# zhuhaozh/metadrive_ped

Measured on AMD Instinct MI355X. Metric: agent-steps/sec at 4096 envs x 240-beam lidar, higher is better.
Workload: dtype f32; 1 GPU; BASELINE configs[1]: 4096 batched MetaDriveEnv per GPU, 3-block PG map (reference default block distribution: curves, straights, ramps, X/T intersections, roundabouts), 240-beam lidar, traffic_density=0.1, trigger traffic, auto-reset; envs_per_gpu=4096, agents_per_env=1, mover_capacity=24, n_beams=240

## Files before the change

### metadrive_ped_amd/csrc/mdstep.hip

```cpp
#include <hip/hip_runtime.h>
#include <stddef.h>
#include <stdint.h>
#include <stdio.h>
#include <stdlib.h>

#include <type_traits>

#include "md_curriculum.h"
#include "md_expert.h"
#include "md_expert_sense.h"
#include "md_ai_protect.h"
#include "md_scenario.h"
#include "md_topdown.h"
#include "md_render.h"
#include "md_branch.h"
#include "md_ped.h"
#include "md_vector_obs.h"
#include "md_lean_pins.h"

namespace {

constexpr int kBlock = 256;

enum Phase : int {
    PH_RESET = 1,
    PH_IDM = 2,
    PH_INTEGRATE = 4,
    PH_LOCALIZE = 8,
    PH_CONTACTS = 16,
    PH_TRAFFIC = 32,
    PH_OBSERVE = 64,
    PH_LIDAR = 128,
    PH_LIFECYCLE = 256,
    PH_ALL = 511,
    PH_LOCALIZE_ROAD_FIRST = PH_LOCALIZE | (1 << 20),
};

thread_local char g_err[256] = "ok";

#ifdef MD_STAMP
__device__ unsigned long long* g_stamp_buf = nullptr;
__device__ const int* g_env_order = nullptr;
#define MD_STAMP_AT(i)                                                                         \
    do {                                                                                       \
        if (threadIdx.x == 0 && g_stamp_buf) {                                                 \
            unsigned long long* sb_ = g_stamp_buf + (size_t)blockIdx.x * 32;                   \
            sb_[(i)] = __builtin_readcyclecounter();                                           \
            if ((i) == 0) {                                                                    \
                sb_[12] = __builtin_amdgcn_s_memrealtime();                                    \
                sb_[14] = (unsigned long long)__builtin_amdgcn_s_getreg(63492) |               \
                          ((unsigned long long)__builtin_amdgcn_s_getreg(63508) << 32);        \
            }                                                                                  \
            if ((i) == 11) sb_[13] = __builtin_amdgcn_s_memrealtime();                         \
        }                                                                                      \
    } while (0)
#define MD_FINE_STAMP(cond, i)                                                                 \
    do {                                                                                       \
        if ((cond) && g_stamp_buf) g_stamp_buf[(size_t)blockIdx.x * 32 + 16 + (i)] = __builtin_readcyclecounter(); \
    } while (0)
#define MD_LOC_COUNT(cond, hit)                                                                \
    do {                                                                                       \
        if ((cond) && g_stamp_buf) {                                                           \
            atomicAdd(&g_stamp_buf[(size_t)blockIdx.x * 32 + 16 + 12], 1ull);                  \
            if (hit) atomicAdd(&g_stamp_buf[(size_t)blockIdx.x * 32 + 16 + 13], 1ull);         \
        }                                                                                      \
    } while (0)
#define MD_AHEAD_STAMP(cond, i)                                                                \
    do {                                                                                       \
        if ((cond) && g_stamp_buf) g_stamp_buf[(size_t)blockIdx.x * 32 + (i)] = __builtin_readcyclecounter(); \
    } while (0)
enum : int { MD_AHEAD_EVALUATED = 32, MD_AHEAD_HIT = 40, MD_AHEAD_MISS = 48 };
#define MD_AHEAD_COUNT(cond, what)                                                             \
    do {                                                                                       \
        if ((cond) && g_stamp_buf) atomicAdd(&g_stamp_buf[(size_t)blockIdx.x * 32 + 16 + 12], 1ull << (what)); \
    } while (0)
__device__ unsigned long long* g_contacts_buf = nullptr;
#define MD_CONTACTS_STAMP(cond, i)                                                             \
    do {                                                                                       \
        if ((cond) && g_contacts_buf) g_contacts_buf[(size_t)blockIdx.x * 8 + (i)] = __builtin_readcyclecounter(); \
    } while (0)
#define MD_CONTACTS_COUNT(cond, cells, items)                                                  \
    do {                                                                                       \
        if ((cond) && g_contacts_buf) {                                                        \
            g_contacts_buf[(size_t)blockIdx.x * 8 + 4] += (unsigned long long)(cells);         \
            g_contacts_buf[(size_t)blockIdx.x * 8 + 5] += (unsigned long long)(items);         \
        }                                                                                      \
    } while (0)
#else
#define MD_CONTACTS_STAMP(cond, i) do { } while (0)
#define MD_CONTACTS_COUNT(cond, cells, items) do { } while (0)
#define MD_STAMP_AT(i) do { } while (0)
#define MD_FINE_STAMP(cond, i) do { } while (0)
#define MD_LOC_COUNT(cond, hit) do { } while (0)
#define MD_AHEAD_STAMP(cond, i) do { } while (0)
#define MD_AHEAD_COUNT(cond, what) do { } while (0)
#endif
#ifndef MD_ENV_SKIP
#define MD_ENV_SKIP 0
#endif

__host__ __device__ constexpr uint32_t align_up(uint32_t b, uint32_t a) { return (b + a - 1) & ~(a - 1); }

__device__ __forceinline__ float bcast_f(float v, int src) { return __shfl(v, src, 64); }
__device__ __forceinline__ int bcast_i(int v, int src) { return __shfl(v, src, 64); }

__device__ __forceinline__ void wave_lds_sync() {
    __builtin_amdgcn_fence(__ATOMIC_RELEASE, "wavefront");
    __builtin_amdgcn_wave_barrier();
    __builtin_amdgcn_fence(__ATOMIC_ACQUIRE, "wavefront");
}

#ifndef MD_NT_STAGE
#define MD_NT_STAGE 1
#endif
typedef unsigned int md_u32x4 __attribute__((ext_vector_type(4)));
__device__ __forceinline__ uint4 ld_stream(const uint4* p) {
#if MD_NT_STAGE
    const md_u32x4 v = __builtin_nontemporal_load(reinterpret_cast<const md_u32x4*>(p));
    return make_uint4(v.x, v.y, v.z, v.w);
#else
    return *p;
#endif
}
__device__ __forceinline__ void st_stream(uint4* p, const uint4 v) {
#if MD_NT_STAGE
    md_u32x4 t;
    t.x = v.x; t.y = v.y; t.z = v.z; t.w = v.w;
    __builtin_nontemporal_store(t, reinterpret_cast<md_u32x4*>(p));
#else
    *p = v;
#endif
}
__device__ __forceinline__ void st_stream_f(float* p, float v) {
#if MD_NT_STAGE
    __builtin_nontemporal_store(v, p);
#else
    *p = v;
#endif
}

__device__ __forceinline__ int wave_min_i(int v, bool valid, int none) {
    unsigned long long m = __ballot(valid);
    int best = none;
    while (m) {
        const int l = __ffsll((long long)m) - 1;
        m &= m - 1;
        const int o = __shfl(v, l, 64);
        best = o < best ? o : best;
    }
    return best;
}

template <bool kLdsRow = false>
__device__ __forceinline__ void lidar_item(const MdWorld& w, const MdState& s, const MdConfig& c, int a, int sec, int lane,
                           float* __restrict__ out_row, unsigned long long* det) {
    const MdShape me = s.shape[a];
    const int beam = sec * 64 + lane;
    const bool valid = beam < c.n_beams;
    if (!md_present(me.flags)) {
        if (valid) out_row[beam] = 1.0f;
        return;
    }
    float bc = 1.0f, bs = 0.0f;
    if (valid) {
        bc = w.beam_cs[2 * beam];
        bs = w.beam_cs[2 * beam + 1];
    }
    const float dirx = (bc * me.c - bs * me.s) * c.lidar_range;
    const float diry = (bs * me.c + bc * me.s) * c.lidar_range;

    const int nb = min(64, c.n_beams - sec * 64);
// ... 272 lines not shown
        for (int fan = 0; fan < (f.n1 > 0 ? 2 : 1); ++fan) {
            const float* beam_cs = fan ? f.cs1 : f.cs0;
            const int n_beams = fan ? f.n1 : f.n0;
            const float reach = (fan ? f.range1 : f.range0) * 1.001f;
            const uint32_t kind_mask = fan ? f.mask1 : f.mask0;
            const float phase0 = fan ? ph1 : ph0;
            const bool uniform_fan = fan ? uni1 : uni0;
            const int beam_base = fan ? f.n0 : 0;
            const float inv_dphi = 1.0f / (6.283185307179586f / (float)n_beams);
            const float far = reach + rr;
            const bool near = in_reach && ((kind_mask >> b.kind) & 1u) && !(px * px + py * py > far * far);
            if (__ballot(near) == 0ull) continue;
            int i_lo = 0, n_try = n_beams;
            if (uniform_fan && near && n_beams > kAllBeamsMax)
                detector_beam_window(me, px, py, rr, phase0, inv_dphi, n_beams, i_lo, n_try);
            const int nt = near ? n_try : 0;
            int pin = nt;
#pragma unroll
            for (int off = 1; off < 64; off <<= 1) {
                const int v = __shfl_up(pin, off, 64);
                if (lane_id >= off) pin += v;
            }
            const int total = __shfl(pin, 63, 64);
            const int pex = pin - nt;
            for (int t0 = 0; t0 < total; t0 += 64) {
                const int t = t0 + lane_id;
                int l = 0;
#pragma unroll
                for (int step = 32; step >= 1; step >>= 1) {
                    const int cnd = l + step;
                    const int pc = __shfl(pex, cnd & 63, 64);
                    if (cnd < 64 && pc <= t) l = cnd;
                }
                const bool mine_ = t < total;
                const int k = t - __shfl(pex, l, 64);
                const float px_ = __shfl(px, l, 64), py_ = __shfl(py, l, 64), rr_ = __shfl(rr, l, 64);
                int i = __shfl(i_lo, l, 64) + k;
                if (i >= n_beams) i -= n_beams;
                if (!mine_) i = 0;
                const int q_ = __shfl(q0, l, 64);
                const float bc = beam_cs[2 * i], bs = beam_cs[2 * i + 1];
                const float ux = bc * me.c - bs * me.s, uy = bs * me.c + bc * me.s;
                const float perp = ux * py_ - uy * px_, along = ux * px_ + uy * py_;
                const bool pass = mine_ && !(md_fabs(perp) > rr_ * 1.001f + 1.0e-3f || along < -rr_ || along > reach + rr_);
                const unsigned long long m = __ballot(pass);
                if (m == 0ull) continue;
                if (cnt + 64 > kPairs) {
                    wave_lds_sync();
                    detector_drain2(w, me, f, pair_list, cnt, qa, lane_id);
                    __builtin_amdgcn_wave_barrier();
                    cnt = 0;
                }
                if (pass) pair_list[cnt + __popcll(m & ((1ull << lane_id) - 1ull))] = ((q_ - qa) << 8) | (beam_base + i);
                cnt += __popcll(m);
            }
        }
    }
    __builtin_amdgcn_wave_barrier();
    n_near = 0;
    };
    for (int q0 = qa; q0 < qb; q0 += 64) {
        const int q = q0 + lane_id;
        const QuadBall b = nb;
        if (q + 64 < qb) nb = quad_ball_of(w, q + 64);
        bool in_reach = false;
        if (q < qb) {
            const float px = b.mx - me.cx, py = b.my - me.cy;
            const float far = reach_max + b.rr;
            in_reach = !(px * px + py * py > far * far);
        }
        const unsigned long long m = __ballot(in_reach);
        if (m == 0ull) continue;
        if (n_near + 64 > kNear) work_off();
        if (in_reach) near_list[n_near + __popcll(m & ((1ull << lane_id) - 1ull))] = q - qa;
        n_near += __popcll(m);
        if (!across_rounds) work_off();
    }
    work_off();
    wave_lds_sync();
    detector_drain2(w, me, f, pair_list, cnt, qa, lane_id);
    __builtin_amdgcn_wave_barrier();
}

__device__ __host__ inline int detector_parts(int A) { return (A >= kBlock / 64) ? 1 : kBlock / 64; }
__device__ __host__ inline int detector_groups(int A) { return (A * detector_parts(A) + kBlock / 64 - 1) / (kBlock / 64); }

struct LineDetectorLds { uint32_t best, beams, pairs, bytes; };
__host__ __device__ inline LineDetectorLds line_detector_lds(int nb) {
    constexpr int kW = kBlock / 64;
    LineDetectorLds L;
    L.best = 0;
    L.beams = L.best + (uint32_t)kW * nb * sizeof(int);
    L.pairs = L.beams + (uint32_t)nb * 2 * sizeof(float);
    L.bytes = L.pairs + (uint32_t)kW * kDetPairs * sizeof(int);
    return L;
}

__global__ __launch_bounds__(kBlock) void line_detector_kernel(MdWorld w, MdState s, MdConfig c,
                                                               const float* __restrict__ beam_cs, int n_beams,
                                                               float range, uint32_t kind_mask, float* out,
                                                               int out_stride, int out_offset,
                                                               const float* __restrict__ beam_cs1, int n_beams1, float range1,
                                                               uint32_t kind_mask1, int out_offset1) {
    extern __shared__ __attribute__((aligned(16))) unsigned char smem[];
    constexpr int kW = kBlock / 64;
    const int A = c.agents_per_env;
    const int nb = n_beams + n_beams1;
    const int parts = detector_parts(A), groups = detector_groups(A);
    const LineDetectorLds L = line_detector_lds(nb);
    int* l_best = reinterpret_cast<int*>(smem + L.best);
    float* l_bm = reinterpret_cast<float*>(smem + L.beams);
    int* l_pairs = reinterpret_cast<int*>(smem + L.pairs);
    const int e = blockIdx.x / groups, grp = blockIdx.x - e * groups;
    if (e >= c.n_envs) return;
    const int tid = threadIdx.x, wave = tid >> 6, lane = tid & 63;
    const int m = w.env_map[e];
    const int q0 = w.quad_off[m], q1 = w.quad_off[m + 1];
    const int a_first = (grp * kW) / parts;
    const int n_here = min(A - a_first, kW / parts);
    for (int it = tid; it < n_here * nb; it += kBlock) l_best[it] = __float_as_int(1.0f);
    for (int it = tid; it < 2 * n_beams; it += kBlock) l_bm[it] = beam_cs[it];
    for (int it = tid; it < 2 * n_beams1; it += kBlock) l_bm[2 * n_beams + it] = beam_cs1[it];
    __syncthreads();
    const int per = (q1 - q0 + parts - 1) / parts;
    const int it = grp * kW + wave;
    if (it < A * parts) {
        const int a = it / parts, part = it - a * parts;
        const MdShape me = s.shape[e * c.cap + a];
        if (md_present(me.flags)) {
            const int qa = q0 + part * per, qb = min(qa + per, q1);
            DetFan2 f;
            f.cs0 = l_bm; f.n0 = n_beams; f.range0 = range; f.mask0 = kind_mask; f.best0 = l_best + (a - a_first) * nb;
            f.cs1 = l_bm + 2 * n_beams; f.n1 = n_beams1; f.range1 = range1; f.mask1 = kind_mask1; f.best1 = f.best0 + n_beams;
            detector_wave2(w, me, qa, qb, f, l_pairs + wave * kDetPairs, lane);
        }
    }
    __syncthreads();
    for (int k = tid; k < n_here * nb; k += kBlock) {
        const int al = k / nb, i = k - al * nb;
        float* row = out + (size_t)(e * A + a_first + al) * out_stride;
        if (i < n_beams) row[out_offset + i] = __int_as_float(l_best[k]);
        else row[out_offset1 + (i - n_beams)] = __int_as_float(l_best[k]);
    }
}

}

#include "parts/localize.inc"
#include "parts/contacts.inc"
#include "parts/idm.inc"
#include "parts/observe.inc"
#include "parts/trigger.inc"
#include "parts/lifecycle.inc"

namespace {

__device__ __forceinline__ void copy16(void* dst, const void* src, int nbytes, int tid, int nthreads) {
    uint4* d = reinterpret_cast<uint4*>(dst);
    const uint4* s = reinterpret_cast<const uint4*>(src);
    for (int i = tid; i < (nbytes >> 4); i += nthreads) d[i] = s[i];
}

constexpr int kStageMaxLanes = 64;
constexpr int kWideMaxEnvs = 640;
constexpr uint32_t kRemovedMark = 0xFFFFFFFFu;

__device__ __forceinline__ int kth_bit(unsigned long long lo, unsigned long long hi, int k) {
    int slot = -1;
    while (k >= 0) {
        if (lo) {
            slot = __ffsll((long long)lo) - 1;
            lo &= lo - 1;
        } else if (hi) {
            slot = 64 + __ffsll((long long)hi) - 1;
            hi &= hi - 1;
        } else {
            return -1;
        }
        --k;
    }
    return slot;
}

struct EnvImage {
    MdShape* shape;
    MdDyn* dyn;
    MdPid* pid;
    MdParam* param;
    MdNav* nav;
    float* action;
    uint32_t* flags;
    int32_t* final_lane;
};

__device__ __forceinline__ MdState local_view(const MdState& gv, const EnvImage& img) {
    MdState s = gv;
    s.shape = img.shape;
    s.dyn = img.dyn;
    s.nav = img.nav;
    s.pid = img.pid;
    s.action = img.action;
    s.flags = img.flags;
    s.param = img.param;
    s.final_lane = img.final_lane;
    return s;
}

struct SlotMask { unsigned long long lo, hi; };
static_assert(MD_MAX_CAP <= 128, "drive_mask: two 64-bit words per env");
__device__ __forceinline__ SlotMask drive_mask(const MdShape* shape, int cap, int lane) {
    SlotMask m = {0ull, 0ull};
    for (int j0 = 0; j0 < cap; j0 += 64) {
        const int j = j0 + lane;
        const unsigned long long mk = __ballot(j < cap && md_drives(shape[j < cap ? j : 0].flags));
        if (j0 == 0) m.lo = mk;
        else m.hi = mk;
    }
    return m;
}
__device__ __forceinline__ SlotMask agent_share(SlotMask m, int agents) {
    m.lo &= agents >= 64 ? ~0ull : ((1ull << agents) - 1ull);
    m.hi &= agents <= 64 ? 0ull : (agents >= 128 ? ~0ull : ((1ull << (agents - 64)) - 1ull));
    return m;
}
__device__ __forceinline__ int popc(SlotMask m) { return __popcll(m.lo) + __popcll(m.hi); }

#ifndef MD_ENV_BLOCK
#define MD_ENV_BLOCK 256
#endif
#ifndef MD_ENV_WAVES_EU
#define MD_ENV_WAVES_EU 7
#endif
__device__ __forceinline__ void lean_pins_fold(MdState& s, MdConfig& c) {
#define MD_PIN_ZERO(f) c.f = 0;
#define MD_PIN_NUL(p) s.p = nullptr;
    MD_LEAN_PINS(MD_PIN_ZERO, MD_PIN_NUL)
#undef MD_PIN_ZERO
#undef MD_PIN_NUL
}
__device__ __forceinline__ void lean_size_pins_fold(MdConfig& c, MdConfig& c_scan) {
#define MD_PIN_EQUALS(f, v) c.f = (v);
#define MD_PIN_AT_MOST(f, v)
    MD_LEAN_SIZE_PINS(MD_PIN_EQUALS, MD_PIN_AT_MOST)
#undef MD_PIN_EQUALS
#undef MD_PIN_AT_MOST
    c_scan = c;
#define MD_PIN_EQUALS(f, v)
#define MD_PIN_AT_MOST(f, v) c_scan.f = min(c.f, (v));
    MD_LEAN_SIZE_PINS(MD_PIN_EQUALS, MD_PIN_AT_MOST)
#undef MD_PIN_EQUALS
#undef MD_PIN_AT_MOST
}

template <int PH, bool RESPAWN, bool MULTI>
constexpr int env_waves_per_eu() { return (PH == PH_ALL && !RESPAWN && !MULTI && MD_ENV_BLOCK >= 128) ? MD_ENV_WAVES_EU : 0; }

struct EnvLds { uint32_t shape, dyn, nav, pid, action, flags, lanes, roads, scratch, param, final_lane, det, onlane, cfl, tk, bytes; };
__host__ __device__ inline EnvLds env_lds(int cap, int agents, int n_lanes, int n_roads, int waves, bool multi, bool lidar_only) {
    EnvLds L;
    L.shape = 0;
    L.dyn = L.shape + (uint32_t)cap * sizeof(MdShape);
    L.nav = L.dyn + (uint32_t)cap * sizeof(MdDyn);
    L.pid = L.nav + (uint32_t)cap * sizeof(MdNav);
    L.action = L.pid + (uint32_t)cap * sizeof(MdPid);
    L.flags = L.action + (uint32_t)cap * 2 * sizeof(float);
    L.lanes = align_up(L.flags + (uint32_t)cap * sizeof(uint32_t), 16);
    L.roads = L.lanes + (uint32_t)n_lanes * sizeof(MdLane);
    L.scratch = L.roads + (uint32_t)n_roads * sizeof(MdRoad);
    L.param = L.scratch + (uint32_t)waves * (multi ? kObsScratch : 48) * sizeof(float);
    L.final_lane = L.param + (uint32_t)cap * sizeof(MdParam);
    L.det = L.final_lane + align_up(cap, 2) * sizeof(int32_t);
    L.onlane = L.det + (uint32_t)agents * 2 * sizeof(unsigned long long);
    L.cfl = L.onlane + (uint32_t)cap * sizeof(uint32_t);
    const uint32_t shared_words = 2 * cap > 8 ? 2 * cap : 8;
    L.tk = L.onlane + shared_words * sizeof(uint32_t);
    L.bytes = lidar_only ? L.dyn : L.tk + 3 * sizeof(int);
    return L;
}

template <int PH, bool STAGE_MAP, bool RESPAWN = false, bool MULTI = false, int BLK = MD_ENV_BLOCK, bool NARROW = false>
__global__ __launch_bounds__(BLK)
__attribute__((amdgpu_waves_per_eu(env_waves_per_eu<PH, RESPAWN, MULTI>() ? env_waves_per_eu<PH, RESPAWN, MULTI>() : 1,
                                   env_waves_per_eu<PH, RESPAWN, MULTI>() ? env_waves_per_eu<PH, RESPAWN, MULTI>() : 8)))
void env_kernel(MdWorld w, MdState g, MdConfig c, float* lidar_out,
                                                  int lidar_stride, int lidar_offset) {
    constexpr int kBlock = BLK;
    constexpr int kWaves = kBlock / 64;
    constexpr bool kIdmKeys = !STAGE_MAP && !RESPAWN && !MULTI;
    constexpr bool kLocRoadFirst = PH == PH_ALL ? kIdmKeys : PH == PH_LOCALIZE_ROAD_FIRST;
    constexpr bool kObsLockstep = MD_OBS_LOCKSTEP && PH == PH_ALL && kIdmKeys;
    constexpr bool kObsAhead = MD_OBS_AHEAD && kObsLockstep && kWaves > 1;
    constexpr bool kContactsFlat = MD_CONTACTS_FLAT && PH == PH_ALL && kIdmKeys;
    if constexpr (PH == PH_ALL && !RESPAWN && !MULTI && !STAGE_MAP) lean_pins_fold(g, c);
    static_assert(!NARROW || (PH == PH_ALL && !RESPAWN && !MULTI && !STAGE_MAP), "NARROW: a form of the lean non-staged kernel only");
    MdConfig c_scan = c;
    if constexpr (NARROW) lean_size_pins_fold(c, c_scan);
    if ((int)blockIdx.x >= c.n_envs) return;
#ifdef MD_STAMP
    const int e = g_env_order ? g_env_order[blockIdx.x] : (int)blockIdx.x;
#else
    const int e = blockIdx.x;
#endif
    const int tid = threadIdx.x;
    const int wave = tid >> 6, lane = tid & 63;
    const int cap = c.cap;

    const int n_stage_lanes = STAGE_MAP ? w.max_lanes : 0, n_stage_roads = STAGE_MAP ? w.max_roads : 0;
    constexpr bool kLidarOnly = (PH == PH_LIDAR);
    const EnvLds L = env_lds(cap, c.agents_per_env, n_stage_lanes, n_stage_roads, kWaves, MULTI, kLidarOnly);
    extern __shared__ __attribute__((aligned(16))) unsigned char smem[];
    MdShape* l_shape = reinterpret_cast<MdShape*>(smem + L.shape);
    MdDyn* l_dyn = reinterpret_cast<MdDyn*>(smem + L.dyn);
    MdNav* l_nav = reinterpret_cast<MdNav*>(smem + L.nav);
    MdPid* l_pid = reinterpret_cast<MdPid*>(smem + L.pid);
    float* l_action = reinterpret_cast<float*>(smem + L.action);
    uint32_t* l_flags = reinterpret_cast<uint32_t*>(smem + L.flags);
    MdLane* l_lanes = reinterpret_cast<MdLane*>(smem + L.lanes);
    MdRoad* l_roads = reinterpret_cast<MdRoad*>(smem + L.roads);
    float* l_scratch = reinterpret_cast<float*>(smem + L.scratch) + wave * (MULTI ? kObsScratch : 48);
    MdParam* l_param = reinterpret_cast<MdParam*>(smem + L.param);
    int32_t* l_final = reinterpret_cast<int32_t*>(smem + L.final_lane);
    unsigned long long* l_det = reinterpret_cast<unsigned long long*>(smem + L.det);
    const EnvImage img = {l_shape, l_dyn, l_pid, l_param, l_nav, l_action, l_flags, l_final};
    uint32_t* l_onlane = reinterpret_cast<uint32_t*>(smem + L.onlane);
    uint32_t* l_cfl = reinterpret_cast<uint32_t*>(smem + L.cfl);
    int* l_tk = reinterpret_cast<int*>(smem + L.tk);
    const bool track_det = (PH == PH_ALL) && (RESPAWN || MULTI) && g.detected != nullptr;

    const MdState gv = md_env_view(&g, &c, e);
    const int reset_flag = (PH & PH_RESET) ? gv.need_reset[0] : 0;

    MD_STAMP_AT(0);
    const bool kFusedAct = (PH == PH_ALL) && gv.agent_action != nullptr;
    const MdLane* lanes;
    const MdRoad* roads;
    if (STAGE_MAP) {
        lanes = l_lanes;
        roads = l_roads;
    } else {
        lanes = w.lanes + w.lane_off[w.env_map[e]];
        roads = w.roads + w.road_off[w.env_map[e]];
    }
    if (kLidarOnly) {
        copy16(l_shape, gv.shape, cap * (int)sizeof(MdShape), tid, kBlock);
    } else if (kBlock >= 256) {
        const int n32 = cap * 2, n64 = cap * 4;
        const uint4* g_shape = reinterpret_cast<const uint4*>(gv.shape);
        const uint4* g_dyn = reinterpret_cast<const uint4*>(gv.dyn);
        const uint4* g_pid = reinterpret_cast<const uint4*>(gv.pid);
        const uint4* g_param = reinterpret_cast<const uint4*>(gv.param);
        const uint4* g_nav = reinterpret_cast<const uint4*>(gv.nav);
        uint4 r_shape, r_dyn, r_pid, r_param, r_nav0;
        float2 r_act;
        uint32_t r_fl;
        int r_fin;
        const bool p32 = tid < n32, pc = tid < cap;
        if (p32) {
            r_shape = ld_stream(&g_shape[tid]);
            r_dyn = ld_stream(&g_dyn[tid]);
            r_pid = ld_stream(&g_pid[tid]);
            r_param = ld_stream(&g_param[tid]);
        }
        if (tid < n64) r_nav0 = ld_stream(&g_nav[tid]);
        if (pc) {
            r_act = (kFusedAct && tid < c.agents_per_env) ? reinterpret_cast<const float2*>(gv.agent_action)[tid]
                                                          : reinterpret_cast<const float2*>(gv.action)[tid];
            r_fl = gv.flags[tid];
            r_fin = gv.final_lane ? gv.final_lane[tid] : 0;
        }
        if (STAGE_MAP) {
            const int m = w.env_map[e];
            const int lo = w.lane_off[m], ro = w.road_off[m];
            copy16(l_lanes, w.lanes + lo, (w.lane_off[m + 1] - lo) * (int)sizeof(MdLane), tid, kBlock);
            copy16(l_roads, w.roads + ro, (w.road_off[m + 1] - ro) * (int)sizeof(MdRoad), tid, kBlock);
        }
        if (p32) {
            reinterpret_cast<uint4*>(l_shape)[tid] = r_shape;
            reinterpret_cast<uint4*>(l_dyn)[tid] = r_dyn;
            reinterpret_cast<uint4*>(l_pid)[tid] = r_pid;
            reinterpret_cast<uint4*>(l_param)[tid] = r_param;
        }
        if (tid < n64) reinterpret_cast<uint4*>(l_nav)[tid] = r_nav0;
        for (int i = tid + kBlock; i < n64; i += kBlock) reinterpret_cast<uint4*>(l_nav)[i] = g_nav[i];
        if (pc) {
            reinterpret_cast<float2*>(l_action)[tid] = r_act;
            l_flags[tid] = r_fl;
            l_final[tid] = r_fin;
        }
        if (track_det)
            for (int j = tid; j < 2 * c.agents_per_env; j += kBlock) l_det[j] = 0ull;
    } else {
        copy16(l_shape, gv.shape, cap * (int)sizeof(MdShape), tid, kBlock);
        if (STAGE_MAP) {
            const int m = w.env_map[e];
            const int lo = w.lane_off[m], ro = w.road_off[m];
            copy16(l_lanes, w.lanes + lo, (w.lane_off[m + 1] - lo) * (int)sizeof(MdLane), tid, kBlock);
            copy16(l_roads, w.roads + ro, (w.road_off[m + 1] - ro) * (int)sizeof(MdRoad), tid, kBlock);
        }
        copy16(l_dyn, gv.dyn, cap * (int)sizeof(MdDyn), tid, kBlock);
        copy16(l_nav, gv.nav, cap * (int)sizeof(MdNav), tid, kBlock);
        copy16(l_pid, gv.pid, cap * (int)sizeof(MdPid), tid, kBlock);
        copy16(l_param, gv.param, cap * (int)sizeof(MdParam), tid, kBlock);
        for (int j = tid; j < cap; j += kBlock) {
            const float* src = (kFusedAct && j < c.agents_per_env) ? gv.agent_action : gv.action;
            l_action[2 * j] = src[2 * j];
            l_action[2 * j + 1] = src[2 * j + 1];
            l_flags[j] = gv.flags[j];
            l_final[j] = gv.final_lane ? gv.final_lane[j] : 0;
        }
        if (track_det)
            for (int j = tid; j < 2 * c.agents_per_env; j += kBlock) l_det[j] = 0ull;
    }
    const bool do_reset = reset_flag != 0;
    const int just_reset = do_reset ? 1 : 0;
    if (do_reset && !kLidarOnly) {
        __syncthreads();
        copy16(l_shape, gv.shape0, cap * (int)sizeof(MdShape), tid, kBlock);
        copy16(l_dyn, gv.dyn0, cap * (int)sizeof(MdDyn), tid, kBlock);
        copy16(l_nav, gv.nav0, cap * (int)sizeof(MdNav), tid, kBlock);
        copy16(l_pid, gv.pid0, cap * (int)sizeof(MdPid), tid, kBlock);
        if (MULTI && c.random_agent_model && gv.param0)
            copy16(l_param, gv.param0, cap * (int)sizeof(MdParam), tid, kBlock);
        for (int j = tid; j < cap; j += kBlock) {
            l_action[2 * j] = 0.0f;
            l_action[2 * j + 1] = 0.0f;
            l_flags[j] = 0u;
        }
        if (MULTI || (RESPAWN && (c.traffic_mode == 1 || c.traffic_mode == 2))) {
            for (int i = tid; i < cap * MD_ROUTE_LEN; i += kBlock) {
                gv.route_nodes[i] = gv.route_nodes0[i];
                gv.route_roads[i] = gv.route_roads0[i];
            }
            for (int j = tid; j < cap; j += kBlock) l_final[j] = gv.final_lane0[j];
        }
        if (MULTI) {
            for (int j = tid; j < cap; j += kBlock) gv.agent_id[j] = j;
            if (tid == 0) {
                gv.env_steps[0] = 0;
                int n0 = 0;
                for (int j = 0; j < c.agents_per_env; ++j) n0 += (gv.shape0[j].flags & MD_F_ALIVE) ? 1 : 0;
                gv.next_agent_id[0] = n0;
            }
        }
    }
    MdState s = local_view(gv, img);
    if (kLidarOnly) {
        s = gv;
        s.shape = l_shape;
    }
    if ((MULTI || PH == PH_ALL) && tid == 0) l_tk[0] = l_tk[1] = l_tk[2] = 0;
    if (kObsAhead && tid == 0) reinterpret_cast<int*>(smem + L.scratch)[kAhMark] = 0;
    __syncthreads();
    MD_STAMP_AT(1);
    constexpr bool kTriggerEarly = MD_TRIGGER_EARLY && PH == PH_ALL && kIdmKeys && kWaves > 1;
    constexpr int kTrigWord = (kWaves - 1) * 48 + 46;
    if (kTriggerEarly && wave == kWaves - 1) {
        int min_order, trig_road;
        trigger_search_wave(s, c_scan, lane, &min_order, &trig_road);
        if (lane == 0) {
            int* l_trig = reinterpret_cast<int*>(smem + L.scratch) + kTrigWord;
            l_trig[0] = min_order;
            l_trig[1] = trig_road;
        }
    }

    if ((PH & PH_LIFECYCLE) && MULTI && !just_reset) {
        lifecycle_block(w, s, c, w.env_map[e], tid, kBlock, reinterpret_cast<int*>(l_onlane));
    }

    constexpr bool kFused = (PH == PH_ALL);
    const bool agent_idm = (kFused && !RESPAWN && !MULTI) ? false : (c.agent_idm == MD_AGENT_IDM);
    const bool lane_change = (RESPAWN || MULTI) && c.agent_idm == MD_AGENT_LANE_CHANGE;
    constexpr bool kPlanAhead = kFused && kWaves > 1 && !MULTI;
    const bool plan_ahead = kPlanAhead && !agent_idm;
    if ((PH & PH_IDM) && !just_reset && !plan_ahead) {
        if (wave == 0) trigger_env(lanes, s, c, lane);
        __syncthreads();
        MD_STAMP_AT(2);
        for (int j = (agent_idm ? 0 : c.agents_per_env) + wave; j < cap; j += kWaves) {
            const int f = s.shape[j].flags;
            if (md_drives(f) && (agent_idm || !(f & MD_F_AGENT))) idm_vehicle_wave<kIdmKeys>(w, lanes, roads, s, c, w.env_map[e], j, lane, reinterpret_cast<int*>(l_scratch));
        }
        __syncthreads();
    }
    MD_STAMP_AT(3);
    if ((PH & PH_INTEGRATE) && !just_reset) {
        for (int j = tid; j < cap; j += kBlock) {
            if (lane_change && j < c.agents_per_env) {
                const int f = s.shape[j].flags;
                if (md_drives(f) && !(f & MD_F_SPAWNED)) md_lane_change_act(lanes, roads, &s, j);
            }
            if (RESPAWN) md_advance_mover(&s, &c, j);
            else md_integrate_mover(&s, &c, j);
        }
        if (!RESPAWN)
            for (int j = tid; j < cap; j += kBlock) md_walk_mover(&s, &c, j);
        __syncthreads();
    }
    MD_STAMP_AT(4);
    unsigned long long drv_lo = 0ull, drv_hi = 0ull;
    if (kFused) {
        const SlotMask drv = drive_mask(s.shape, cap, lane);
        drv_lo = drv.lo;
        drv_hi = NARROW ? 0ull : drv.hi;
        const SlotMask adrv = agent_share(drv, c.agents_per_env);
        const unsigned long long adrv_lo = adrv.lo, adrv_hi = NARROW ? 0ull : adrv.hi;
        const int nd = NARROW ? __popcll(drv_lo) : popc(drv), na = NARROW ? __popcll(adrv_lo) : popc(adrv);
        if (MULTI) {
            const int npair = (nd + 1) >> 1;
            for (int guard = 0; guard < npair + na; ++guard) {
                int item = 0;
                if (lane == 0) item = atomicAdd(&l_tk[0], 1);
                item = __builtin_amdgcn_readfirstlane(item);
                if (item < 0 || item >= npair + na) break;
                if (item < na) contacts_vehicle(w, s, c, e, kth_bit(adrv_lo, adrv_hi, item), lane, l_cfl);
                else localize_pair(w, lanes, roads, s, e, kth_bit(drv_lo, drv_hi, 2 * (item - na)), kth_bit(drv_lo, drv_hi, 2 * (item - na) + 1), lane, l_onlane);
            }
        } else if (nd + na <= kWaves) {
            for (int item = wave; item < nd + na; item += kWaves) {
                if (item < nd) {
                    if (!(MD_ENV_SKIP & 4)) localize_vehicle<kLocRoadFirst>(w, lanes, roads, s, e, kth_bit(drv_lo, drv_hi, item), lane, l_onlane);
                } else if (!(MD_ENV_SKIP & 8)) contacts_vehicle<kContactsFlat>(w, s, c, e, kth_bit(adrv_lo, adrv_hi, item - nd), lane, l_cfl);
            }
            if constexpr (kObsAhead) {
                if (nd + na < kWaves && wave == nd + na && !(MD_ENV_SKIP & 16))
                    observe_ahead_wave(lanes, roads, s, c, lane, reinterpret_cast<float*>(smem + L.scratch));
            }
        } else {
            const int npair = (nd + 1) >> 1;
            for (int item = wave; item < npair + na; item += kWaves) {
                if (item < npair) {
                    if (!(MD_ENV_SKIP & 4)) localize_pair<kLocRoadFirst>(w, lanes, roads, s, e, kth_bit(drv_lo, drv_hi, 2 * item), kth_bit(drv_lo, drv_hi, 2 * item + 1), lane, l_onlane);
                } else if (!(MD_ENV_SKIP & 8))
                    contacts_vehicle<kContactsFlat>(w, s, c, e, kth_bit(adrv_lo, adrv_hi, item - npair), lane, l_cfl);
            }
        }
        __syncthreads();
    } else {
        if (PH & PH_LOCALIZE) {
            for (int j = wave; j < cap; j += kWaves) localize_vehicle<kLocRoadFirst>(w, lanes, roads, s, e, j, lane);
            __syncthreads();
        }
        MD_STAMP_AT(5);
        if (PH & PH_CONTACTS) {
            for (int j = wave; j < cap; j += kWaves) contacts_vehicle(w, s, c, e, j, lane);
            __syncthreads();
        }
    }
    MD_STAMP_AT(6);
    if (PH & PH_TRAFFIC) {
        for (int j = tid; j < cap; j += kBlock) {
            const bool drove = kFused ? ((((j < 64) ? (drv_lo >> j) : (drv_hi >> (j - 64))) & 1ull) != 0ull) : false;
            if (kFused && !drove) continue;
            const int f = s.shape[j].flags;
            if (kFused)
                s.flags[j] = l_onlane[j] | ((f & MD_F_AGENT) ? l_cfl[j] : 0u);
            if (md_drives(f) && !(f & MD_F_AGENT) && !(s.flags[j] & MD_FL_ON_LANE)) {
                s.shape[j].flags = f & ~MD_F_ALIVE;
                if (kFused) l_cfl[j] = kRemovedMark;
            }
        }
        if (plan_ahead && wave == kWaves - 1) {
            if (kTriggerEarly) {
                const int* l_trig = reinterpret_cast<const int*>(smem + L.scratch) + kTrigWord;
                trigger_fire_wave(lanes, s, c_scan, lane, __builtin_amdgcn_readfirstlane(l_trig[0]), __builtin_amdgcn_readfirstlane(l_trig[1]));
            } else trigger_env(lanes, s, c_scan, lane);
        }
        __syncthreads();
        if (RESPAWN) {
            if (tid == 0) md_traffic_respawn_env(&w, lanes, &s, &c, w.env_map[e]);
            __syncthreads();
        }
    }
    MD_STAMP_AT(7);
    if (plan_ahead) {
        if (wave == 0) {
            if (!(MD_ENV_SKIP & 16))
                for (int a = 0; a < c.agents_per_env; ++a) observe_agent_wave1<kObsLockstep, kObsAhead>(lanes, roads, s, c, a, just_reset, lane, l_scratch);
        } else if (!(MD_ENV_SKIP & 2)) {
            int rank = 0;
            for (int j0 = 0; j0 < cap; j0 += 64) {
                const int jl = j0 + lane;
                const int fl = (jl < cap) ? s.shape[jl].flags : 0;
                unsigned long long mk = __ballot(jl < cap && md_drives(fl) && !(fl & MD_F_AGENT));
                while (mk) {
                    const int j = j0 + __ffsll((long long)mk) - 1;
                    mk &= mk - 1;
                    if (rank % (kWaves - 1) == wave - 1) idm_vehicle_wave<kIdmKeys>(w, lanes, roads, s, c_scan, w.env_map[e], j, lane, reinterpret_cast<int*>(l_scratch));
                    ++rank;
                }
            }
        }
        MD_STAMP_AT(8);
    } else if (PH & PH_OBSERVE) {
        if (MULTI) {
            const int n_grp = (c.agents_per_env + kObsGroups - 1) / kObsGroups;
            for (int guard = 0; guard < n_grp; ++guard) {
                int gi = 0;
                if (lane == 0) gi = atomicAdd(&l_tk[1], 1);
                gi = __builtin_amdgcn_readfirstlane(gi);
                if (gi < 0 || gi >= n_grp) break;
                observe_agent_wave(lanes, roads, s, c, gi * kObsGroups, just_reset, lane, l_scratch);
            }
        } else {
            for (int a = wave; a < c.agents_per_env; a += kWaves) observe_agent_wave1(lanes, roads, s, c, a, just_reset, lane, l_scratch);
        }
        MD_STAMP_AT(8);
    }
    if ((PH & PH_LIDAR) && !(PH == PH_ALL && (MD_ENV_SKIP & 1))) {
        if (c.n_beams > 0) phase_lidar(w, s, c_scan, e, tid, kWaves, lidar_out, lidar_stride, lidar_offset, track_det ? l_det : nullptr, PH == PH_ALL ? &l_tk[2] : nullptr);
    }

    MD_STAMP_AT(9);
    if (!kLidarOnly) {
        __syncthreads();
        MD_STAMP_AT(10);
        constexpr bool respawns = (PH & PH_TRAFFIC) && RESPAWN;
        if (kFused && !MULTI && !do_reset) {
            const bool replay = c.traffic_mode == 3;
            auto dirty = [&](int j) { return replay || md_moves(l_shape[j].flags) || l_cfl[j] == kRemovedMark; };
            for (int i = tid; i < cap * 2; i += kBlock)
                if (dirty(i >> 1)) {
                    st_stream(&reinterpret_cast<uint4*>(gv.shape)[i], reinterpret_cast<const uint4*>(l_shape)[i]);
                    st_stream(&reinterpret_cast<uint4*>(gv.dyn)[i], reinterpret_cast<const uint4*>(l_dyn)[i]);
                    st_stream(&reinterpret_cast<uint4*>(gv.pid)[i], reinterpret_cast<const uint4*>(l_pid)[i]);
                }
            for (int i = tid; i < cap * 4; i += kBlock)
                if (dirty(i >> 2)) st_stream(&reinterpret_cast<uint4*>(gv.nav)[i], reinterpret_cast<const uint4*>(l_nav)[i]);
            for (int j = tid; j < cap; j += kBlock)
                if (dirty(j)) {
                    reinterpret_cast<float2*>(gv.action)[j] = reinterpret_cast<const float2*>(l_action)[j];
                    gv.flags[j] = l_flags[j];
                    if (RESPAWN) gv.final_lane[j] = l_final[j];
                }
            if (track_det)
                for (int j = tid; j < 2 * c.agents_per_env; j += kBlock) gv.detected[j] = l_det[j];
            MD_STAMP_AT(11);
            return;
        }
        if (PH & (PH_RESET | PH_IDM | PH_INTEGRATE | PH_TRAFFIC | PH_OBSERVE | PH_LIFECYCLE)) copy16(gv.shape, l_shape, cap * (int)sizeof(MdShape), tid, kBlock);
        if (MULTI && (PH & (PH_RESET | PH_LIFECYCLE)) && c.random_agent_model && c.is_multi_agent)
            copy16(gv.param, l_param, cap * (int)sizeof(MdParam), tid, kBlock);
        if ((PH & (PH_RESET | PH_INTEGRATE | PH_LIFECYCLE)) || respawns) copy16(gv.dyn, l_dyn, cap * (int)sizeof(MdDyn), tid, kBlock);
        if ((PH & (PH_RESET | PH_IDM | PH_LOCALIZE | PH_OBSERVE | PH_LIFECYCLE)) || respawns) copy16(gv.nav, l_nav, cap * (int)sizeof(MdNav), tid, kBlock);
        if ((PH & (PH_RESET | PH_IDM | PH_OBSERVE | PH_LIFECYCLE)) || respawns || (lane_change && (PH & PH_INTEGRATE)))
            copy16(gv.pid, l_pid, cap * (int)sizeof(MdPid), tid, kBlock);
        if (((PH & (PH_RESET | PH_LIFECYCLE)) && MULTI) || ((PH & (PH_RESET | PH_TRAFFIC)) && RESPAWN)) {
            for (int j = tid; j < cap; j += kBlock) gv.final_lane[j] = l_final[j];
        }
        for (int j = tid; j < cap; j += kBlock) {
            if ((PH & (PH_RESET | PH_IDM | PH_INTEGRATE | PH_LIFECYCLE)) || respawns) {
                gv.action[2 * j] = l_action[2 * j];
                gv.action[2 * j + 1] = l_action[2 * j + 1];
            }
            if ((PH & (PH_RESET | PH_LOCALIZE | PH_CONTACTS | PH_OBSERVE | PH_LIFECYCLE)) || respawns) gv.flags[j] = l_flags[j];
        }
        if (track_det)
            for (int j = tid; j < 2 * c.agents_per_env; j += kBlock) gv.detected[j] = l_det[j];
        if (do_reset && tid == 0) gv.need_reset[0] = 0;
    }
    MD_STAMP_AT(11);
}

#ifndef MD_WAVE_ENVS
#define MD_WAVE_ENVS 4
#endif
constexpr int kWaveEnvs = MD_WAVE_ENVS;

struct WaveEnvLds { uint32_t shape, dyn, pid, param, nav, action, flags, final_lane, onlane, cfl, scratch, det, bytes; };
__host__ __device__ inline WaveEnvLds wave_env_lds(int cap, int agents) {
    WaveEnvLds L;
    L.shape = 0;
    L.dyn = L.shape + (uint32_t)cap * sizeof(MdShape);
    L.pid = L.dyn + (uint32_t)cap * sizeof(MdDyn);
    L.param = L.pid + (uint32_t)cap * sizeof(MdPid);
    L.nav = L.param + (uint32_t)cap * sizeof(MdParam);
    L.action = L.nav + (uint32_t)cap * sizeof(MdNav);
    L.flags = L.action + (uint32_t)cap * 2 * sizeof(float);
    L.final_lane = L.flags + (uint32_t)cap * sizeof(uint32_t);
    L.onlane = L.final_lane + (uint32_t)cap * sizeof(int32_t);
    L.cfl = L.onlane + (uint32_t)cap * sizeof(uint32_t);
    L.scratch = L.cfl + (uint32_t)cap * sizeof(uint32_t);
    L.det = L.scratch + 48 * sizeof(float);
    L.bytes = align_up(L.det + (uint32_t)agents * 2 * sizeof(unsigned long long), 16);
    return L;
}
static_assert((sizeof(MdShape) + sizeof(MdDyn) + sizeof(MdPid) + sizeof(MdParam) + sizeof(MdNav) + 6 * 4) % 8 == 0 && 48 * 4 % 8 == 0,
              "wave_env_lds: the detected sets need 8-B alignment");

template <bool RESPAWN>
__global__ __launch_bounds__(64 * kWaveEnvs) void wave_step_kernel(MdWorld w, MdState g, MdConfig c, float* lidar_out,
                                                                  int lidar_stride, int lidar_offset) {
    if constexpr (!RESPAWN) lean_pins_fold(g, c);
    const int lane = threadIdx.x & 63;
    const int e = blockIdx.x * (blockDim.x >> 6) + (threadIdx.x >> 6);
    if (e >= c.n_envs) return;
    const int cap = c.cap;
    const int A = c.agents_per_env;

    extern __shared__ __attribute__((aligned(16))) unsigned char smem[];
    const WaveEnvLds L = wave_env_lds(cap, A);
    unsigned char* base = smem + __builtin_amdgcn_readfirstlane(threadIdx.x >> 6) * L.bytes;
    MdShape* l_shape = reinterpret_cast<MdShape*>(base + L.shape);
    MdDyn* l_dyn = reinterpret_cast<MdDyn*>(base + L.dyn);
    MdPid* l_pid = reinterpret_cast<MdPid*>(base + L.pid);
    MdParam* l_param = reinterpret_cast<MdParam*>(base + L.param);
    MdNav* l_nav = reinterpret_cast<MdNav*>(base + L.nav);
    float* l_action = reinterpret_cast<float*>(base + L.action);
    uint32_t* l_flags = reinterpret_cast<uint32_t*>(base + L.flags);
    int32_t* l_final = reinterpret_cast<int32_t*>(base + L.final_lane);
    uint32_t* l_onlane = reinterpret_cast<uint32_t*>(base + L.onlane);
    uint32_t* l_cfl = reinterpret_cast<uint32_t*>(base + L.cfl);
    float* l_scratch = reinterpret_cast<float*>(base + L.scratch);
    unsigned long long* l_det = reinterpret_cast<unsigned long long*>(base + L.det);
    const EnvImage img = {l_shape, l_dyn, l_pid, l_param, l_nav, l_action, l_flags, l_final};
    const bool track_det = RESPAWN && g.detected != nullptr;

    const MdState gv = md_env_view(&g, &c, e);
    const int reset_flag = gv.need_reset[0];
    MD_STAMP_AT(0);
    const int m = w.env_map[e];
    const MdLane* lanes = w.lanes + w.lane_off[m];
    const MdRoad* roads = w.roads + w.road_off[m];
    const bool fused_act = gv.agent_action != nullptr;

    {
        const int n32 = cap * 2, n64 = cap * 4;
        const uint4* g_shape = reinterpret_cast<const uint4*>(gv.shape);
        const uint4* g_dyn = reinterpret_cast<const uint4*>(gv.dyn);
        const uint4* g_pid = reinterpret_cast<const uint4*>(gv.pid);
        const uint4* g_param = reinterpret_cast<const uint4*>(gv.param);
        const uint4* g_nav = reinterpret_cast<const uint4*>(gv.nav);
        uint4 r_shape, r_dyn, r_pid, r_param, r_nav0, r_nav1;
        float2 r_act;
        uint32_t r_fl;
        int r_fin;
        const bool p32 = lane < n32, pc = lane < cap;
        if (p32) {
            r_shape = ld_stream(&g_shape[lane]);
            r_dyn = ld_stream(&g_dyn[lane]);
            r_pid = ld_stream(&g_pid[lane]);
            r_param = ld_stream(&g_param[lane]);
        }
        if (lane < n64) r_nav0 = ld_stream(&g_nav[lane]);
        if (lane + 64 < n64) r_nav1 = ld_stream(&g_nav[lane + 64]);
        if (pc) {
            r_act = (fused_act && lane < A) ? reinterpret_cast<const float2*>(gv.agent_action)[lane]
                                            : reinterpret_cast<const float2*>(gv.action)[lane];
            r_fl = gv.flags[lane];
            r_fin = gv.final_lane ? gv.final_lane[lane] : 0;
        }
        if (p32) {
            reinterpret_cast<uint4*>(l_shape)[lane] = r_shape;
            reinterpret_cast<uint4*>(l_dyn)[lane] = r_dyn;
            reinterpret_cast<uint4*>(l_pid)[lane] = r_pid;
            reinterpret_cast<uint4*>(l_param)[lane] = r_param;
        }
        if (lane < n64) reinterpret_cast<uint4*>(l_nav)[lane] = r_nav0;
        if (lane + 64 < n64) reinterpret_cast<uint4*>(l_nav)[lane + 64] = r_nav1;
        if (pc) {
            reinterpret_cast<float2*>(l_action)[lane] = r_act;
            l_flags[lane] = r_fl;
            l_final[lane] = r_fin;
        }
        for (int i = lane + 64; i < n32; i += 64) {
            reinterpret_cast<uint4*>(l_shape)[i] = g_shape[i];
            reinterpret_cast<uint4*>(l_dyn)[i] = g_dyn[i];
            reinterpret_cast<uint4*>(l_pid)[i] = g_pid[i];
            reinterpret_cast<uint4*>(l_param)[i] = g_param[i];
        }
// ... 1459 lines not shown
```

Before: 64.01 million agent-steps/s.

## Lazily re-read kernel arguments from kernarg segment to cut live SGPRs

In the lean fused env kernel, the large by-value world, state and config structs are zeroed, and only the fields each phase needs are reloaded from the kernarg segment pointer right where they are used: stage-in, reset, observe, lidar and write-back. Opaque asm barriers keep the compiler from hoisting these loads back to kernel entry. The aim is to shorten scalar register live ranges across the long kernel, reducing register pressure or spills and possibly allowing higher occupancy. In exchange it adds repeated scalar loads. It also risks missing a config field that some path reads from the zeroed structs, since the config is only partly reconstructed.

```diff
diff --git a/include/md_lean_view.h b/include/md_lean_view.h
--- /dev/null
+++ b/include/md_lean_view.h
@@ -0,0 +1,33 @@
+#ifndef MD_LEAN_VIEW_H
+#define MD_LEAN_VIEW_H
+
+#include <stddef.h>
+
+#include "mdstep.h"
+
+typedef struct MdStepArgs {
+    MdWorld w;
+    MdState g;
+    MdConfig c;
+    float* lidar_out;
+    int32_t lidar_stride;
+    int32_t lidar_offset;
+} MdStepArgs;
+
+#define MD_STEP_ARGS(X) X(w) X(g) X(c) X(lidar_out) X(lidar_stride) X(lidar_offset)
+
+#define MD_LEAN_ARGS_STAGE_IN(X) \
+    X(c.n_envs) X(c.agents_per_env) X(c.cap) \
+    X(g.shape) X(g.dyn) X(g.pid) X(g.param) X(g.nav) X(g.action) X(g.agent_action) X(g.flags) X(g.final_lane) X(g.need_reset) \
+    X(w.env_map) X(w.lane_off) X(w.lanes) X(w.road_off) X(w.roads)
+   
+#define MD_LEAN_ARGS_WRITE_BACK(X) X(g.shape) X(g.dyn) X(g.pid) X(g.nav) X(g.action) X(g.flags) X(g.need_reset)
+#define MD_LEAN_ARGS_RESET(X) X(g.shape0) X(g.dyn0) X(g.nav0) X(g.pid0)
+#define MD_LEAN_ARGS_OBSERVE(X) X(g.obs) X(g.reward) X(g.cost) X(g.step_info) X(g.done_out) X(g.need_reset)
+#define MD_LEAN_ARGS_ROUTES(X) X(g.route_nodes) X(g.route_roads) X(g.idm_rand) X(g.rng)
+#define MD_LEAN_ARGS_LIDAR(X) X(lidar_out) X(lidar_stride) X(lidar_offset)
+#define MD_LEAN_ARGS(X) \
+    MD_LEAN_ARGS_STAGE_IN(X) MD_LEAN_ARGS_WRITE_BACK(X) MD_LEAN_ARGS_RESET(X) MD_LEAN_ARGS_OBSERVE(X) MD_LEAN_ARGS_ROUTES(X) \
+    MD_LEAN_ARGS_LIDAR(X)
+
+#endif
diff --git a/metadrive_ped_amd/csrc/mdstep.hip b/metadrive_ped_amd/csrc/mdstep.hip
--- a/metadrive_ped_amd/csrc/mdstep.hip
+++ b/metadrive_ped_amd/csrc/mdstep.hip
@@ -17,6 +17,7 @@
 #include "md_ped.h"
 #include "md_vector_obs.h"
 #include "md_lean_pins.h"
+#include "md_lean_view.h"
 
 namespace {
 
@@ -595,6 +596,7 @@
 #include "parts/observe.inc"
 #include "parts/trigger.inc"
 #include "parts/lifecycle.inc"
+#include "parts/lean_view.inc"
 
 namespace {
 
@@ -734,6 +736,17 @@
     constexpr bool kObsLockstep = MD_OBS_LOCKSTEP && PH == PH_ALL && kIdmKeys;
     constexpr bool kObsAhead = MD_OBS_AHEAD && kObsLockstep && kWaves > 1;
     constexpr bool kContactsFlat = MD_CONTACTS_FLAT && PH == PH_ALL && kIdmKeys;
+    constexpr bool kLeanView = MD_LEAN_VIEW && PH == PH_ALL && kIdmKeys && BLK >= 256;
+    LeanStageIn lean_in;
+    if constexpr (kLeanView) {
+        lean_in = lean_stage_in_args(lean_args_entry());
+        w = MdWorld{};
+        g = MdState{};
+        c = MdConfig{};
+        c.n_envs = lean_in.n_envs;
+        c.cap = lean_in.cap;
+        c.agents_per_env = lean_in.agents;
+    }
     if constexpr (PH == PH_ALL && !RESPAWN && !MULTI && !STAGE_MAP) lean_pins_fold(g, c);
     static_assert(!NARROW || (PH == PH_ALL && !RESPAWN && !MULTI && !STAGE_MAP), "NARROW: a form of the lean non-staged kernel only");
     MdConfig c_scan = c;
@@ -770,17 +783,18 @@
     int* l_tk = reinterpret_cast<int*>(smem + L.tk);
     const bool track_det = (PH == PH_ALL) && (RESPAWN || MULTI) && g.detected != nullptr;
 
-    const MdState gv = md_env_view(&g, &c, e);
+    MdState gv = md_env_view(&g, &c, e);
+    const MdLane* lanes;
+    const MdRoad* roads;
+    if constexpr (kLeanView) lean_view_stage_in(gv, lean_in, e, cap, c.agents_per_env);
     const int reset_flag = (PH & PH_RESET) ? gv.need_reset[0] : 0;
 
     MD_STAMP_AT(0);
     const bool kFusedAct = (PH == PH_ALL) && gv.agent_action != nullptr;
-    const MdLane* lanes;
-    const MdRoad* roads;
     if (STAGE_MAP) {
         lanes = l_lanes;
         roads = l_roads;
-    } else {
+    } else if constexpr (!kLeanView) {
         lanes = w.lanes + w.lane_off[w.env_map[e]];
         roads = w.roads + w.road_off[w.env_map[e]];
     }
@@ -811,21 +825,37 @@
             r_fl = gv.flags[tid];
             r_fin = gv.final_lane ? gv.final_lane[tid] : 0;
         }
+        if constexpr (kLeanView) {
+            lean_view_map(&lanes, &roads, lean_args_entry(), e);
+            const LeanArgs kb = lean_args_here();
+            const int n_envs = c.n_envs, agents = c.agents_per_env;
+            lean_arg_copy(w, kb, offsetof(MdStepArgs, w));
+            lean_arg_copy(c, kb, offsetof(MdStepArgs, c));
+            c.n_envs = n_envs;
+            c.cap = cap;
+            c.agents_per_env = agents;
+            lean_pins_fold(g, c);
+            c_scan = c;
+            if constexpr (NARROW) lean_size_pins_fold(c, c_scan);
+            lean_view_routes(gv, kb, e, cap);
+        }
         if (STAGE_MAP) {
             const int m = w.env_map[e];
             const int lo = w.lane_off[m], ro = w.road_off[m];
             copy16(l_lanes, w.lanes + lo, (w.lane_off[m + 1] - lo) * (int)sizeof(MdLane), tid, kBlock);
             copy16(l_roads, w.roads + ro, (w.road_off[m + 1] - ro) * (int)sizeof(MdRoad), tid, kBlock);
         }
-        if (p32) {
+        int tid_st = tid;
+        if constexpr (kLeanView) asm("" : "+v"(tid_st));
+        if (tid_st < n32) {
             reinterpret_cast<uint4*>(l_shape)[tid] = r_shape;
             reinterpret_cast<uint4*>(l_dyn)[tid] = r_dyn;
             reinterpret_cast<uint4*>(l_pid)[tid] = r_pid;
             reinterpret_cast<uint4*>(l_param)[tid] = r_param;
         }
-        if (tid < n64) reinterpret_cast<uint4*>(l_nav)[tid] = r_nav0;
+        if (tid_st < n64) reinterpret_cast<uint4*>(l_nav)[tid] = r_nav0;
         for (int i = tid + kBlock; i < n64; i += kBlock) reinterpret_cast<uint4*>(l_nav)[i] = g_nav[i];
-        if (pc) {
+        if (tid_st < cap) {
             reinterpret_cast<float2*>(l_action)[tid] = r_act;
             l_flags[tid] = r_fl;
             l_final[tid] = r_fin;
@@ -858,6 +888,7 @@
     const int just_reset = do_reset ? 1 : 0;
     if (do_reset && !kLidarOnly) {
         __syncthreads();
+        if constexpr (kLeanView) lean_view_reset(gv, e, cap);
         copy16(l_shape, gv.shape0, cap * (int)sizeof(MdShape), tid, kBlock);
         copy16(l_dyn, gv.dyn0, cap * (int)sizeof(MdDyn), tid, kBlock);
         copy16(l_nav, gv.nav0, cap * (int)sizeof(MdNav), tid, kBlock);
@@ -1018,7 +1049,21 @@
     MD_STAMP_AT(7);
     if (plan_ahead) {
         if (wave == 0) {
-            if (!(MD_ENV_SKIP & 16))
+            if constexpr (kLeanView) {
+                const LeanArgs ko = lean_args_here();
+                MdConfig co;
+                lean_arg_copy(co, ko, offsetof(MdStepArgs, c));
+                co.n_envs = c.n_envs;
+                co.cap = cap;
+                co.agents_per_env = c.agents_per_env;
+                MdConfig co_scan;
+                lean_pins_fold(g, co);
+                if constexpr (NARROW) lean_size_pins_fold(co, co_scan);
+                MdState so = s;
+                lean_view_observe(so, ko, e, co.agents_per_env, co.obs_dim);
+                if (!(MD_ENV_SKIP & 16))
+                    for (int a = 0; a < co.agents_per_env; ++a) observe_agent_wave1<kObsLockstep, kObsAhead>(lanes, roads, so, co, a, just_reset, lane, l_scratch);
+            } else if (!(MD_ENV_SKIP & 16))
                 for (int a = 0; a < c.agents_per_env; ++a) observe_agent_wave1<kObsLockstep, kObsAhead>(lanes, roads, s, c, a, just_reset, lane, l_scratch);
         } else if (!(MD_ENV_SKIP & 2)) {
             int rank = 0;
@@ -1051,6 +1096,12 @@
         MD_STAMP_AT(8);
     }
     if ((PH & PH_LIDAR) && !(PH == PH_ALL && (MD_ENV_SKIP & 1))) {
+        if constexpr (kLeanView) {
+            const LeanArgs kl = lean_args_here();
+            lidar_out = LEAN_ARG(kl, lidar_out);
+            lidar_stride = LEAN_ARG(kl, lidar_stride);
+            lidar_offset = LEAN_ARG(kl, lidar_offset);
+        }
         if (c.n_beams > 0) phase_lidar(w, s, c_scan, e, tid, kWaves, lidar_out, lidar_stride, lidar_offset, track_det ? l_det : nullptr, PH == PH_ALL ? &l_tk[2] : nullptr);
     }
 
@@ -1059,6 +1110,7 @@
         __syncthreads();
         MD_STAMP_AT(10);
         constexpr bool respawns = (PH & PH_TRAFFIC) && RESPAWN;
+        if constexpr (kLeanView) lean_view_write_back(gv, e, cap);
         if (kFused && !MULTI && !do_reset) {
             const bool replay = c.traffic_mode == 3;
             auto dirty = [&](int j) { return replay || md_moves(l_shape[j].flags) || l_cfl[j] == kRemovedMark; };
diff --git a/metadrive_ped_amd/csrc/parts/lean_view.inc b/metadrive_ped_amd/csrc/parts/lean_view.inc
--- /dev/null
+++ b/metadrive_ped_amd/csrc/parts/lean_view.inc
@@ -0,0 +1,117 @@
+
+namespace {
+
+#ifndef MD_LEAN_VIEW
+#define MD_LEAN_VIEW 1
+#endif
+
+typedef const __attribute__((address_space(4))) unsigned char* LeanArgs;
+
+__device__ __forceinline__ LeanArgs lean_args_entry() { return (LeanArgs)__builtin_amdgcn_kernarg_segment_ptr(); }
+__device__ __forceinline__ LeanArgs lean_args_here() {
+    LeanArgs p = lean_args_entry();
+    asm volatile("" : "+s"(p));
+    return p;
+}
+__device__ __forceinline__ int lean_here(int v) {
+    v = __builtin_amdgcn_readfirstlane(v);
+    asm volatile("" : "+s"(v));
+    return v;
+}
+template <typename T>
+__device__ __forceinline__ T lean_arg_at(LeanArgs p, size_t off) {
+    static_assert(std::is_scalar<T>::value, "lean_arg_at: one pointer or number; lean_arg_copy for a struct");
+    return *reinterpret_cast<const __attribute__((address_space(4))) T*>(p + off);
+}
+#define LEAN_ARG(p, field) lean_arg_at<decltype(static_cast<MdStepArgs*>(nullptr)->field)>((p), offsetof(MdStepArgs, field))
+template <typename T>
+__device__ __forceinline__ void lean_arg_copy(T& dst, LeanArgs p, size_t off) {
+    __builtin_memcpy(&dst, reinterpret_cast<const __attribute__((address_space(4))) T*>(p + off), sizeof(T));
+}
+
+
+struct LeanStageIn {
+    int n_envs, agents, cap;
+    MdShape* shape; MdDyn* dyn; MdPid* pid; MdParam* param; MdNav* nav; float* action; const float* agent_action;
+    uint32_t* flags; int32_t* final_lane; int32_t* need_reset;
+};
+__device__ __forceinline__ LeanStageIn lean_stage_in_args(LeanArgs p) {
+    LeanStageIn a;
+    a.n_envs = LEAN_ARG(p, c.n_envs);
+    a.agents = LEAN_ARG(p, c.agents_per_env);
+    a.cap = LEAN_ARG(p, c.cap);
+    a.shape = LEAN_ARG(p, g.shape);
+    a.dyn = LEAN_ARG(p, g.dyn);
+    a.pid = LEAN_ARG(p, g.pid);
+    a.param = LEAN_ARG(p, g.param);
+    a.nav = LEAN_ARG(p, g.nav);
+    a.action = LEAN_ARG(p, g.action);
+    a.agent_action = LEAN_ARG(p, g.agent_action);
+    a.flags = LEAN_ARG(p, g.flags);
+    a.final_lane = LEAN_ARG(p, g.final_lane);
+    a.need_reset = LEAN_ARG(p, g.need_reset);
+    asm("" : "+s"(a.n_envs), "+s"(a.agents), "+s"(a.cap)
+           : "s"(a.shape), "s"(a.dyn), "s"(a.pid), "s"(a.param), "s"(a.nav), "s"(a.action), "s"(a.agent_action), "s"(a.flags), "s"(a.final_lane),
+             "s"(a.need_reset));
+    return a;
+}
+__device__ __forceinline__ void lean_view_stage_in(MdState& v, const LeanStageIn& a, int e, int cap, int agents) {
+    const size_t b = (size_t)e * (size_t)cap;
+    v.shape = a.shape + b;
+    v.dyn = a.dyn + b;
+    v.pid = a.pid + b;
+    v.param = a.param + b;
+    v.nav = a.nav + b;
+    v.action = a.action + 2 * b;
+    v.agent_action = a.agent_action ? a.agent_action + (size_t)e * agents * 2 : nullptr;
+    v.flags = a.flags + b;
+    v.final_lane = a.final_lane ? a.final_lane + b : nullptr;
+    v.need_reset = a.need_reset + e;
+}
+__device__ __forceinline__ void lean_view_map(const MdLane** lanes, const MdRoad** roads, LeanArgs p, int e) {
+    const int m = LEAN_ARG(p, w.env_map)[e];
+    *lanes = LEAN_ARG(p, w.lanes) + LEAN_ARG(p, w.lane_off)[m];
+    *roads = LEAN_ARG(p, w.roads) + LEAN_ARG(p, w.road_off)[m];
+}
+__device__ __forceinline__ void lean_view_write_back(MdState& v, int e, int cap) {
+    const LeanArgs p = lean_args_here();
+    e = lean_here(e);
+    const size_t b = (size_t)e * (size_t)cap;
+    v.shape = LEAN_ARG(p, g.shape) + b;
+    v.dyn = LEAN_ARG(p, g.dyn) + b;
+    v.pid = LEAN_ARG(p, g.pid) + b;
+    v.nav = LEAN_ARG(p, g.nav) + b;
+    v.action = LEAN_ARG(p, g.action) + 2 * b;
+    v.flags = LEAN_ARG(p, g.flags) + b;
+    v.need_reset = LEAN_ARG(p, g.need_reset) + e;
+}
+__device__ __forceinline__ void lean_view_reset(MdState& v, int e, int cap) {
+    const LeanArgs p = lean_args_here();
+    e = lean_here(e);
+    const size_t b = (size_t)e * (size_t)cap;
+    v.shape0 = LEAN_ARG(p, g.shape0) + b;
+    v.dyn0 = LEAN_ARG(p, g.dyn0) + b;
+    v.nav0 = LEAN_ARG(p, g.nav0) + b;
+    v.pid0 = LEAN_ARG(p, g.pid0) + b;
+}
+__device__ __forceinline__ void lean_view_observe(MdState& v, LeanArgs p, int e, int agents, int obs_dim) {
+    e = lean_here(e);
+    const size_t a = (size_t)e * (size_t)agents;
+    v.obs = LEAN_ARG(p, g.obs) + a * (size_t)obs_dim;
+    v.reward = LEAN_ARG(p, g.reward) + a;
+    v.cost = LEAN_ARG(p, g.cost) + a;
+    v.step_info = LEAN_ARG(p, g.step_info) + a * 8;
+    uint8_t* done_out = LEAN_ARG(p, g.done_out);
+    v.done_out = done_out ? done_out + 4 * a : nullptr;
+    v.need_reset = LEAN_ARG(p, g.need_reset) + e;
+}
+__device__ __forceinline__ void lean_view_routes(MdState& v, LeanArgs p, int e, int cap) {
+    const size_t b = (size_t)e * (size_t)cap;
+    v.route_nodes = LEAN_ARG(p, g.route_nodes) + b * MD_ROUTE_LEN;
+    v.route_roads = LEAN_ARG(p, g.route_roads) + b * MD_ROUTE_LEN;
+    v.idm_rand = LEAN_ARG(p, g.idm_rand) + b * MD_IDM_RAND;
+    uint32_t* rng = LEAN_ARG(p, g.rng);
+    v.rng = rng ? rng + e : nullptr;
+}
+
+}
```

Result: faster. 67.27 million agent-steps/s (median of 6 runs) (+5.1%).
